# aszepieniec/stark-brainfuck

Hardware: AMD Instinct MI355X
Metric: goldilocks_ntt_field_elements_per_sec (higher is better)
Workload: dtype u64 (mod 2^64-2^32+1); 1 GPU; forward NTT of 8 independent 2^24-point base-field columns resident in HBM (BASELINE config 5); log_n=24, total_columns=8

## Files before the change

### stark_brainfuck_amd/csrc/ntt.hip

```cpp
#include <cstdio>
#include <cstdlib>
#include <cstring>
#include <vector>

#define BFS_GL_SUB4
#include "runtime.hpp"

namespace bfs {

template <int B1, int B2, int B3, int LOGC, int MODE, bool NT>
__global__ void __launch_bounds__(256) ntt_tile_kernel(const PassArgs a) {
    extern __shared__ __attribute__((aligned(16))) u64 smem[];
    typedef TileCfg<B1, B2, B3, LOGC, MODE> Cfg;
    u64* tw = smem + (B2 > 0 ? ((Cfg::LDS_WORDS + 1) & ~1) : 0);
    static_assert(B1 == 4, "one sub-group of 16 elements per thread");
    constexpr u32 TW_N = Cfg::U >= 2 ? (1u << (B1 + B2)) : 0;
    const u64* tab = a.tw1;
    const u32 tw_shift = a.tb.t_in_log - (B1 + B2);
    const u32 tid = threadIdx.x;
    const u64* lrow = tile_load_row<Cfg, LOGC, MODE>(a, blockIdx.x);
    const u64* srow_g = tile_store_row<Cfg, LOGC, MODE>(a, blockIdx.x);
    const u64* row = lrow ? lrow : srow_g;
    const bool has_row = row != nullptr;
    u64 tw0 = 0, rw0 = 0;
    if (TW_N && tid < TW_N) tw0 = tab[(u64)tid << tw_shift];
    if (has_row && tid < (1u << Cfg::S)) rw0 = row[tid];
    u64 x[16];
    ntt_stage1_load<B1, B2, B3, LOGC, MODE, NT>(a, tid, blockIdx.x, blockIdx.y, 0, x);
    u64* rw = tw + Cfg::TW_WORDS;
    if (TW_N && tid < TW_N) tw[tid] = tw0;
    if (has_row && tid < (1u << Cfg::S)) rw[tid] = rw0;
    for (u32 i = tid + blockDim.x; i < TW_N; i += blockDim.x) tw[i] = tab[(u64)i << tw_shift];
    if (has_row)
        for (u32 i = tid + blockDim.x; i < (1u << Cfg::S); i += blockDim.x) rw[i] = row[i];
    const u64* rowtw = lrow ? rw : nullptr;
    const u64* srow = srow_g && !lrow ? rw : nullptr;
    if (Cfg::U >= 2 || has_row) __syncthreads();
    ntt_stage1_compute<B1, B2, B3, LOGC, MODE, NT>(a, smem, tw, rowtw, threadIdx.x, blockIdx.x, blockIdx.y, 0, x, srow);
    if constexpr (B2 > 0) {
        __syncthreads();
        ntt_stage2<B1, B2, B3, LOGC, MODE, NT>(a, smem, threadIdx.x, blockIdx.x, blockIdx.y, srow);
    }
    if constexpr (B3 > 0) {
        __syncthreads();
        ntt_stage3<B1, B2, B3, LOGC, MODE, NT>(a, smem, threadIdx.x, blockIdx.x, blockIdx.y, srow);
    }
}

#ifndef BFS_NTT_SPLIT_WAVES
#define BFS_NTT_SPLIT_WAVES 6
#endif
template <int B1, int B2, int B3, int LOGC, int MODE, bool NT>
__global__ void __launch_bounds__(256, B2 >= 3 ? BFS_NTT_SPLIT_WAVES : 0) ntt_tile_kernel_split(const PassArgs a) {
    static_assert(B1 == 4 && B2 > 0 && B3 == 0, "two register stages, 16 elements per thread");
    extern __shared__ __attribute__((aligned(16))) u64 smem[];
    typedef TileCfg<B1, B2, B3, LOGC, MODE> Cfg;
    constexpr u32 TILE_BYTES = (Cfg::LDS_WORDS * 4 + 15) & ~15u;
    u32* tile = (u32*)smem;
    u64* tw = (u64*)((char*)smem + TILE_BYTES);
    constexpr u32 TW_N = 1u << (B1 + B2);
    const u64* tab = a.tw1;
    const u32 tw_shift = a.tb.t_in_log - (B1 + B2);
    const u32 tid = threadIdx.x;
    const u32 bx = blockIdx.x, by = blockIdx.y;
    const u64* lrow = tile_load_row<Cfg, LOGC, MODE>(a, bx);
    const u64* srow_g = tile_store_row<Cfg, LOGC, MODE>(a, bx);
    const u64* row = lrow ? lrow : srow_g;
    const bool has_row = row != nullptr;
    u64 tw0 = 0, rw0 = 0;
    if (tid < TW_N) tw0 = tab[(u64)tid << tw_shift];
    if (has_row && tid < (1u << Cfg::S)) rw0 = row[tid];
    u64 x[16];
    ntt_stage1_load<B1, B2, B3, LOGC, MODE, NT>(a, tid, bx, by, 0, x);
    u64* rw = tw + Cfg::TW_WORDS;
    if (tid < TW_N) tw[tid] = tw0;
// ... 12 lines not shown
        for (int d = 0; d < Q2; ++d) lo[s * Q2 + d] = tile[stage2_in_index<B1, B2, B3, LOGC, MODE>(tid, s, d)];
    __syncthreads();
    BFS_UNROLL
    for (int m = 0; m < 16; ++m) tile[stage1_out_index<B1, B2, B3, LOGC, MODE>(a, tid, 0, m)] = (u32)(x[m] >> 32);
    __syncthreads();
    BFS_UNROLL
    for (int s = 0; s < SG2; ++s) {
        u64 y[Q2];
        BFS_UNROLL
        for (int d = 0; d < Q2; ++d) y[d] = ((u64)tile[stage2_in_index<B1, B2, B3, LOGC, MODE>(tid, s, d)] << 32) | lo[s * Q2 + d];
        ntt_stage2_from<B1, B2, B3, LOGC, MODE, NT>(a, smem, tid, bx, by, s, y, srow);
    }
}

__global__ void ntt_small_kernel(const SmallArgs a) { ntt_small_body(a, threadIdx.x, blockIdx.y); }

template <int B1, int B2, int B3, int LOGC, int MODE>
static int launch_tile(TileShape<B1, B2, B3, LOGC, MODE>, const PassArgs& a, u32 grid_x, u32 batch, hipStream_t stream) {
    typedef TileCfg<B1, B2, B3, LOGC, MODE> Cfg;
    const size_t row_words = (a.tb.row != nullptr || a.tb.srow != nullptr) ? (1u << Cfg::S) : 0;
    if constexpr (MODE == PASS_SINGLE) {
        const size_t lds = (size_t)((B2 > 0 ? ((Cfg::LDS_WORDS + 1) & ~1) + Cfg::TW_WORDS : 0) + row_words) * sizeof(u64);
        if (a.streaming)
            hipLaunchKernelGGL((ntt_tile_kernel<B1, B2, B3, LOGC, MODE, true>), dim3(grid_x, batch), dim3(Cfg::W), lds, stream, a);
        else
            hipLaunchKernelGGL((ntt_tile_kernel<B1, B2, B3, LOGC, MODE, false>), dim3(grid_x, batch), dim3(Cfg::W), lds, stream, a);
    } else {
        const size_t lds = ((Cfg::LDS_WORDS * 4 + 15) & ~15u) + (Cfg::TW_WORDS + row_words) * sizeof(u64);
        if (a.streaming)
            hipLaunchKernelGGL((ntt_tile_kernel_split<B1, B2, B3, LOGC, MODE, true>), dim3(grid_x, batch), dim3(Cfg::W), lds, stream, a);
        else
            hipLaunchKernelGGL((ntt_tile_kernel_split<B1, B2, B3, LOGC, MODE, false>), dim3(grid_x, batch), dim3(Cfg::W), lds, stream, a);
    }
    BFS_HIP(hipGetLastError());
    return BFS_OK;
}

enum { TBL_W_LO = 1, TBL_W_HI, TBL_T_IN, TBL_T_IN_LAST, TBL_S_LO, TBL_S_HI, TBL_ROW };

static int get_row_tables(const NttPlan& p, u32 t, u64 root, const u64** d_row, const u64** d_srow) {
    *d_row = nullptr;
    *d_srow = nullptr;
    NttRowSpec load, store;
    ntt_row_specs(p, t, root, load, store);
    for (int which = 0; which < 2; ++which) {
        const NttRowSpec& sp = which ? store : load;
        if (sp.omega == 0) continue;
        const u64** out = which ? d_srow : d_row;
        const u64 key = ((u64)sp.a_bits << 24) | ((u64)sp.b_bits << 16) | TBL_ROW;
        if (cached_table_lookup(sp.omega, key, 0, out)) continue;
        std::vector<u64> host;
        ntt_product_table(sp.omega, sp.a_bits, sp.b_bits, host);
        BFS_TRY(cached_table(sp.omega, key, 0, host.data(), host.size(), out));
    }
    return BFS_OK;
// ... 15 lines not shown
        BFS_TRY(cached_table(root, kb | TBL_T_IN, 0, ht.t_in.data(), ht.t_in.size(), &tb.t_in));
        BFS_TRY(cached_table(root, kb | TBL_T_IN_LAST, post_scale, ht.t_in_last.data(), ht.t_in_last.size(), &tb.t_in_last));
    }
    if (shift != 1) {
        if (!(cached_table_lookup(shift, kb | TBL_S_LO, 0, &tb.s_lo) && cached_table_lookup(shift, kb | TBL_S_HI, 0, &tb.s_hi))) {
            CosetHostTables ct;
            ntt_build_coset_tables(p, shift, ct);
            BFS_TRY(cached_table(shift, kb | TBL_S_LO, 0, ct.s_lo.data(), ct.s_lo.size(), &tb.s_lo));
            BFS_TRY(cached_table(shift, kb | TBL_S_HI, 0, ct.s_hi.data(), ct.s_hi.size(), &tb.s_hi));
        }
    }
    return BFS_OK;
}

int ntt_power_tables(u64 root, u32 log_n, const u64** lo, const u64** hi, u32* lo_bits) {
    NttPlan p;
    if (!ntt_make_plan(log_n, root, p)) { set_error("no table plan for log_n = %u", log_n); return BFS_ERR_BAD_ARG; }
    NttTables tb;
    BFS_TRY(get_tables(p, root, 1, 1, tb));
    *lo = tb.w_lo; *hi = tb.w_hi; *lo_bits = tb.lo_bits;
    return BFS_OK;
}

int ntt_run_steps(const NttCall& c, const NttPlan& p, u64* mid, u32 first, u32 last) {
    NttTables tb;
    BFS_TRY(get_tables(p, c.root, c.shift, c.post_scale, tb));
    const NttSchedule s = ntt_make_schedule(p, c.n_in, mid != nullptr);
    const struct { u64* ptr; u64 stride; } buf[3] = {{const_cast<u64*>(c.in), c.in_stride}, {c.out, c.out_stride}, {mid, 1ull << p.log_n}};
    for (u32 k = first; k <= last && k < s.nsteps; ++k) {
        const NttStep& st = s.step[k];
        BFS_TRY(get_row_tables(p, st.pass, c.root, &tb.row, &tb.srow));
        PassArgs a = ntt_pass_args(p, st.pass, buf[st.src].ptr, buf[st.dst].ptr, buf[st.src].stride, buf[st.dst].stride, st.count, tb, c.shift != 1, c.shift, c.post_scale);
        a.streaming = c.streaming;
        const int rc = ntt_with_tile_shape(st.mode, st.S, [&](auto shape) { return launch_tile(shape, a, st.grid_x, c.batch, c.stream); });
        if (rc == BFS_ERR_BAD_ARG) set_error("internal: no tile kernel for a %u-bit digit in mode %u", st.S, st.mode);
        BFS_TRY(rc);
    }
    return BFS_OK;
}

const NttEnv& ntt_env() {
    static const NttEnv env = [] {
        NttEnv v{NttRouteMode::Remembered, NTT_ROUTE_DIRECT, false, -1, true, false};
        if (const char* e = getenv("BFS_NTT_WS_PROBE")) {
            if (e[0] == '0' || !strcmp(e, "direct")) v.route_mode = NttRouteMode::Forced;
            else if (!strncmp(e, "buffer", 6) && e[6] >= '0' && e[6] < '0' + NTT_ROUTE_CANDIDATES && !e[7]) { v.route_mode = NttRouteMode::Forced; v.forced_route = e[6] - '0'; }
            else if (!strcmp(e, "auto") || !strcmp(e, "1")) v.route_mode = NttRouteMode::Auto;
        }
        if (const char* e = getenv("BFS_NTT_WS_PROBE_LOG")) v.probe_log = e[0] == '1';
        if (const char* e = getenv("BFS_NTT_STREAMING")) v.force_streaming = atoi(e);
        if (const char* e = getenv("BFS_NTT_EXPAND")) v.allow_expand = e[0] != '0';
        v.plan_log = getenv("BFS_NTT_PLAN_LOG") != nullptr;
        return v;
    }();
    return env;
}

int ntt_launch(const u64* d_in, u64 n_in, u64 in_stride, u64* d_out, u64 out_stride, u32 log_n, u32 batch, u64 root,
               u64 shift, u64 post_scale, hipStream_t stream) {
    if (log_n > 32) { set_error("field has no 2^%u-th root of unity (algebra.py:124-125)", log_n); return BFS_ERR_BAD_ARG; }
    const u64 n = 1ull << log_n;
    if (n_in > n) { set_error("more coefficients (%llu) than the evaluation order (%llu)", (unsigned long long)n_in, (unsigned long long)n); return BFS_ERR_TOO_MANY_COEFFS; }
    if (batch == 0) return BFS_OK;
    if (d_out == nullptr || (d_in == nullptr && n_in != 0)) { set_error("bfs_gl_ntt: null device pointer"); return BFS_ERR_BAD_ARG; }
    if (batch > 1 && (out_stride < n || in_stride < n_in)) {
        set_error("bfs_gl_ntt: transforms of a batch overlap (in_stride %llu < %llu coefficients or out_stride %llu < n = %llu)",
                  (unsigned long long)in_stride, (unsigned long long)n_in, (unsigned long long)out_stride, (unsigned long long)n);
        return BFS_ERR_BAD_ARG;
    }
    if (log_n <= NTT_TILE_LOG && n_in != 0) {
        if (ntt_buffers_overlap(d_in, n_in, in_stride, d_out, n, out_stride, batch) && !(d_in == d_out && in_stride == out_stride)) {
            void* w = nullptr;
            const size_t span = (size_t)((u64)(batch - 1) * in_stride + n_in) * sizeof(u64);
            BFS_TRY(workspace(0, span, stream, &w));
            BFS_HIP(hipMemcpyAsync(w, d_in, span, hipMemcpyDeviceToDevice, stream));
// ... 2 lines not shown
    }
    if (batch > 65535) {
        for (u32 done = 0; done < batch;) {
            const u32 part = batch - done < 65535 ? batch - done : 65535;
            BFS_TRY(ntt_launch(d_in + (u64)done * in_stride, n_in, in_stride, d_out + (u64)done * out_stride, out_stride, log_n, part, root,
                               shift, post_scale, stream));
            done += part;
        }
        return BFS_OK;
    }
    int rc = ntt_check_root(root, log_n);
    if (rc == BFS_ERR_NOT_ROOT) { set_error("primitive root must be nth root of unity, where n is %llu", (unsigned long long)n); return rc; }
    if (rc == BFS_ERR_NOT_PRIMITIVE) { set_error("primitive root %llu is not primitive nth root of unity, where n is %llu", (unsigned long long)root, (unsigned long long)n); return rc; }
    const NttEnv& env = ntt_env();
    const bool overlap = log_n > NTT_TILE_LOG && n_in != 0 && ntt_buffers_overlap(d_in, n_in, in_stride, d_out, n, out_stride, batch);
    NttPlan p;
    if (!ntt_choose_plan(log_n, n_in, root, overlap, env.allow_expand, p)) { set_error("no NTT plan for log_n = %u", log_n); return BFS_ERR_BAD_ARG; }
    if (p.npass == 0) {
        SmallArgs a{d_in, d_out, in_stride, out_stride, n_in, log_n, root, shift, post_scale};
        hipLaunchKernelGGL(ntt_small_kernel, dim3(1, batch), dim3(64), 0, stream, a);
        BFS_HIP(hipGetLastError());
        return BFS_OK;
    }
    const u32 streaming = env.force_streaming >= 0 ? (u32)(env.force_streaming != 0) : (u32)((u64)n * batch * sizeof(u64) > NTT_STREAMING_BYTES);
    const NttCall c{d_in, n_in, in_stride, d_out, out_stride, batch, root, shift, post_scale, streaming, stream};
    if (env.plan_log) fprintf(stderr, "ntt plan: log_n %u n_in %llu batch %u overlap %d allow %d in %p out %p\n", log_n, (unsigned long long)n_in, batch, (int)overlap, (int)env.allow_expand, (const void*)d_in, (void*)d_out);
    int route = NTT_ROUTE_DIRECT;
    if (!overlap && !p.expand && p.npass > 1) BFS_TRY(ntt_route(c, p, &route));
    u64* mid = nullptr;
    if (overlap || route >= 0) {
        void* w = nullptr;
        BFS_TRY(workspace(route >= 0 ? NTT_ROUTE_SLOT0 + route : 0, (size_t)n * batch * sizeof(u64), stream, &w));
        mid = (u64*)w;
    }
    return ntt_run_steps(c, p, mid, 0, 3);
}

}
```

### stark_brainfuck_amd/csrc/ntt_core.hpp

```cpp
#pragma once
#include "gl.hpp"

namespace bfs {

constexpr u64 cx_mulmod(u64 a, u64 b) { return (u64)(((u128)a * b) % GL_P); }
constexpr u64 cx_pow2(int k) {
    u64 r = 1;
    for (int i = 0; i < k; ++i) r = cx_mulmod(r, 2);
    return r;
}

template <int K>
BFS_HD u64 mul_pow2(u64 x) {
    static_assert(K >= 0 && K < 96, "rotation amount");
    constexpr int q = K / 32, r = K % 32;
    if constexpr (K == 0) {
        return x;
    } else if constexpr (q == 0) {
        return gl_reduce96((u32)(x >> (64 - r)), x << r);
    } else {
        const u32 x0 = (u32)x, x1 = (u32)(x >> 32);
        u32 y0 = x0, y1 = x1, y2 = 0;
        if constexpr (r != 0) {
            y0 = x0 << r;
// ... 42 lines not shown
}
template <int Q, int LIVE, bool OUT_LAZY>
BFS_HD void dif_sparse(u64* x) {
    if constexpr (Q >= 2) {
        if constexpr (LIVE > Q / 2) {
            dif<Q, OUT_LAZY>(x);
        } else {
            dif_sparse_level<Q, LIVE, OUT_LAZY>(x);
            dif_sparse<Q / 2, LIVE, OUT_LAZY>(x);
            dif_sparse<Q / 2, LIVE, OUT_LAZY>(x + Q / 2);
        }
    }
}

constexpr u32 cx_bitrev(u32 v, int bits) {
    u32 r = 0;
    for (int i = 0; i < bits; ++i) r |= ((v >> i) & 1u) << (bits - 1 - i);
    return r;
}

template <int BITS>
BFS_HD u32 perm_digit(int m, u32 uinv) { return (cx_bitrev((u32)m, BITS) * uinv) & ((1u << BITS) - 1); }

template <bool NT>
BFS_HD u64 ntt_ld(const u64* p) {
#if defined(__HIP_DEVICE_COMPILE__)
    if constexpr (NT) return __builtin_nontemporal_load(p);
#endif
    return *p;
}
template <bool NT>
BFS_HD void ntt_st(u64* p, u64 v) {
#if defined(__HIP_DEVICE_COMPILE__)
    if constexpr (NT) { __builtin_nontemporal_store(v, p); return; }
#endif
    *p = v;
}

struct NttTables {
    const u64* w_lo;
    const u64* w_hi;
    u32 lo_bits;
    u32 t_in_log;
    const u64* t_in;
    const u64* t_in_last;
    const u64* s_lo;
    const u64* s_hi;
    const u64* row;
    const u64* srow;
};

enum { PASS_COLUMN = 0, PASS_SINGLE = 1, PASS_FIRST = 2, PASS_EXPAND = 3 };

struct PassArgs {
    const u64* in;
    u64* out;
    u64 in_batch_stride, out_batch_stride;
// ... 111 lines not shown
template <typename Cfg, int LOGC, int MODE>
BFS_HD const u64* tile_store_row(const PassArgs& a, u32 bid_x) {
    if constexpr (MODE != PASS_FIRST) return nullptr;
    if (a.tb.srow == nullptr) return nullptr;
    const u64 c0 = (u64)(bid_x & ((1u << a.lognl) - 1)) << LOGC;
    const u64 j1 = c0 >> (a.logL - pass_bits_of(a.pass_bits, 1));
    return a.tb.srow + (j1 << Cfg::S);
}

template <int B1, int B2, int B3, int LOGC, int MODE>
BFS_HD void stage2_pos(u32 G, u32& c, u32& f1, u32& f3) {
    if constexpr (MODE == PASS_FIRST) {
        f1 = G & ((1u << B1) - 1);
        c = (G >> B1) & ((1u << LOGC) - 1);
        f3 = G >> (B1 + LOGC);
    } else {
        c = G & ((1u << LOGC) - 1);
        const u32 rest = G >> LOGC;
        f1 = rest & ((1u << B1) - 1);
        f3 = rest >> B1;
    }
}

template <typename Cfg, int LOGC, int MODE, int BQ, bool NT = false>
BFS_HD void final_store(const PassArgs& a, const TileGeom& g, const u64* x, u32 klow, int kshift, u32 c, const u64* srow = nullptr) {
    constexpr int Q = 1 << BQ;
    const bool scale = (Cfg::U == 1) && a.post_scale != 1;
    u64* tp;
    u32 step_log;
    if constexpr (MODE == PASS_COLUMN || MODE == PASS_EXPAND) {
        tp = g.out + g.row0 + ((u64)klow << a.logL) + c;
        step_log = (u32)kshift + a.logL;
    } else if constexpr (MODE == PASS_FIRST) {
        tp = g.out + (digit_reverse(g.c0 + c, a.pass_bits, 1, (int)a.npass - 1) << Cfg::S) + klow;
        step_log = (u32)kshift;
    } else {
        tp = g.out + klow;
        step_log = (u32)kshift;
    }
    BFS_UNROLL
    for (int m = 0; m < Q; ++m) {
        u64 v = scale ? gl_mul(x[m], a.post_scale) : x[m];
        if (srow != nullptr) v = gl_mul(v, srow[klow + (perm_digit<BQ>(m, a.uinv) << kshift)]);
        ntt_st<NT>(tp + ((u64)perm_digit<BQ>(m, a.uinv) << step_log), v);
    }
}

// ... 7 lines not shown
template <int B1, int B2, int B3, int LOGC, int MODE>
BFS_HD void stage1_oc(u32 tid, int sub, u32& o, u32& c) {
    typedef TileCfg<B1, B2, B3, LOGC, MODE> Cfg;
    const u32 G = (u32)sub * Cfg::W + tid;
    c = G & ((1u << LOGC) - 1);
    o = G >> LOGC;
}

template <int B1, int B2, int B3, int LOGC, int MODE>
BFS_HD Stage1Pos<B1, B2, B3, LOGC, MODE> stage1_pos(const PassArgs& a, const TileGeom& g, u32 tid, int sub) {
    typedef TileCfg<B1, B2, B3, LOGC, MODE> Cfg;
    Stage1Pos<B1, B2, B3, LOGC, MODE> p;
    stage1_oc<B1, B2, B3, LOGC, MODE>(tid, sub, p.o, p.c);
    if constexpr (MODE != PASS_SINGLE) {
        p.idx0 = g.row0 + ((u64)p.o << a.logL) + p.c;
        p.step_log = Cfg::SH1 + a.logL;
    } else {
        p.idx0 = p.o;
        p.step_log = Cfg::SH1;
    }
    return p;
}

template <int B1, int B2, int B3, int LOGC, int MODE, bool NT = false>
BFS_HD void ntt_stage1_load(const PassArgs& a, u32 tid, u32 bid_x, u32 bid_y, int sub, u64* x) {
    typedef TileCfg<B1, B2, B3, LOGC, MODE> Cfg;
    constexpr int Q = 1 << B1;
    const TileGeom g = tile_geom<Cfg, LOGC, MODE>(a, bid_x, bid_y);
    const Stage1Pos<B1, B2, B3, LOGC, MODE> p = stage1_pos<B1, B2, B3, LOGC, MODE>(a, g, tid, sub);
    if constexpr (MODE == PASS_EXPAND) {
        const u64 i0 = ((u64)p.o << a.tw_shift) + g.h;
        const u32 sl = Cfg::SH1 + a.tw_shift;
        const u64* ip = a.in + (u64)bid_y * a.in_batch_stride + i0;
        BFS_UNROLL
        for (int d = 0; d < Q; ++d) x[d] = (i0 + ((u64)d << sl) < a.n_main) ? ntt_ld<NT>(ip + ((u64)d << sl)) : 0;
        return;
    }
    const u64* tp = g.in + p.idx0;
    if (a.partial) {
        BFS_UNROLL
        for (int d = 0; d < Q; ++d) x[d] = (p.idx0 + ((u64)d << p.step_log) < a.n_in) ? ntt_ld<NT>(tp + ((u64)d << p.step_log)) : 0;
    } else {
        BFS_UNROLL
        for (int d = 0; d < Q; ++d) x[d] = ntt_ld<NT>(tp + ((u64)d << p.step_log));
    }
}

template <int B1, int B2, int B3, int LOGC, int MODE>
BFS_HD u32 stage1_out_index(const PassArgs& a, u32 tid, int sub, int m) {
    typedef TileCfg<B1, B2, B3, LOGC, MODE> Cfg;
    u32 o, c;
    stage1_oc<B1, B2, B3, LOGC, MODE>(tid, sub, o, c);
    return lds_addr<Cfg, LOGC>((perm_digit<B1>(m, a.uinv) << Cfg::SH1) | o, c);
}

template <int B1, int B2, int B3, int LOGC, int MODE>
BFS_HD u32 stage2_in_index(u32 tid, int s, int d) {
    typedef TileCfg<B1, B2, B3, LOGC, MODE> Cfg;
    u32 c, f1, f3;
    stage2_pos<B1, B2, B3, LOGC, MODE>((u32)s * Cfg::W + tid, c, f1, f3);
    return lds_addr<Cfg, LOGC>((f1 << Cfg::SH1) | ((u32)d << Cfg::SH2) | f3, c);
}

template <int B1, int B2, int B3, int LOGC, int MODE, bool NT = false>
BFS_HD void ntt_stage1_values(const PassArgs& a, const u64* tw, const u64* rowtw, u32 tid, u32 bid_x, u32 bid_y, int sub, u64* x,
                              const u64* srow = nullptr) {
    typedef TileCfg<B1, B2, B3, LOGC, MODE> Cfg;
    constexpr int Q = 1 << B1;
    const TileGeom g = tile_geom<Cfg, LOGC, MODE>(a, bid_x, bid_y);
    const u64 nmask = (1ull << a.log_n) - 1;
    const Stage1Pos<B1, B2, B3, LOGC, MODE> p = stage1_pos<B1, B2, B3, LOGC, MODE>(a, g, tid, sub);
    const u32 o = p.o, c = p.c;
    u32 dmax = Q;
    if constexpr (MODE == PASS_EXPAND) {
        const u32 sl = Cfg::SH1 + a.tw_shift;
        const u64 live = (a.n_main + ((1ull << sl) - 1)) >> sl;
        if (live < (u64)Q) dmax = (u32)live;
    } else if (a.partial) {
        const u64 live = (a.n_in + ((1ull << p.step_log) - 1)) >> p.step_log;
        if (live < (u64)Q) dmax = (u32)live;
    }
    if constexpr (MODE == PASS_EXPAND) {
        const u64 i0 = ((u64)o << a.tw_shift) + g.h;
        if (a.extras != 0 && i0 < (u64)a.extras) {
            const u64 e = g.in[(1ull << a.main_bits) + i0];
            u64 f = tw_pow(a.tb.w_lo, a.tb.w_hi, a.tb.lo_bits, ((g.c0 + c) << a.main_bits) & nmask);
            if (a.has_coset) f = gl_mul(f, a.extra_scale);
// ... 37 lines not shown
            if (dmax <= 1) dif_sparse<16, 1, (Cfg::U >= 2)>(x);
            else if (dmax <= 2) dif_sparse<16, 2, (Cfg::U >= 2)>(x);
            else if (dmax <= 4) dif_sparse<16, 4, (Cfg::U >= 2)>(x);
            else dif_sparse<16, 8, (Cfg::U >= 2)>(x);
        }
    } else {
        dif<Q, (Cfg::U >= 2)>(x);
    }
    if constexpr (Cfg::U == 1) {
        final_store<Cfg, LOGC, MODE, B1, NT>(a, g, x, 0, 0, c, srow);
    } else {
        const u32 i2 = o >> B3;
        BFS_UNROLL
        for (int m = 0; m < Q; ++m) {
            const u32 k1 = perm_digit<B1>(m, a.uinv);
            const u32 e = mul24(i2, k1) & ((1u << (B1 + B2)) - 1);
            const bool unit = (m == 0) && a.unit0;
            if (!unit) x[m] = gl_mul(x[m], tw[e]);
            else x[m] = gl_canon(x[m]);
        }
    }
}

template <int B1, int B2, int B3, int LOGC, int MODE, bool NT = false>
BFS_HD void ntt_stage1_compute(const PassArgs& a, u64* smem, const u64* tw, const u64* rowtw, u32 tid, u32 bid_x, u32 bid_y, int sub, u64* x,
                               const u64* srow = nullptr) {
    typedef TileCfg<B1, B2, B3, LOGC, MODE> Cfg;
    ntt_stage1_values<B1, B2, B3, LOGC, MODE, NT>(a, tw, rowtw, tid, bid_x, bid_y, sub, x, srow);
    if constexpr (Cfg::U >= 2) {
        BFS_UNROLL
        for (int m = 0; m < (1 << B1); ++m) smem[stage1_out_index<B1, B2, B3, LOGC, MODE>(a, tid, sub, m)] = x[m];
    }
}

template <int B1, int B2, int B3, int LOGC, int MODE>
BFS_HD void ntt_stage1(const PassArgs& a, u64* smem, const u64* tw, const u64* rowtw, u32 tid, u32 bid_x, u32 bid_y, const u64* srow = nullptr) {
    constexpr int Q = 1 << B1, SG = 16 / Q;
    BFS_UNROLL
    for (int s = 0; s < SG; ++s) {
        u64 x[Q];
        ntt_stage1_load<B1, B2, B3, LOGC, MODE>(a, tid, bid_x, bid_y, s, x);
        ntt_stage1_compute<B1, B2, B3, LOGC, MODE>(a, smem, tw, rowtw, tid, bid_x, bid_y, s, x, srow);
    }
}

template <int B1, int B2, int B3, int LOGC, int MODE, bool NT = false>
BFS_HD void ntt_stage2_from(const PassArgs& a, u64* smem, u32 tid, u32 bid_x, u32 bid_y, int s, u64* x, const u64* srow = nullptr) {
    typedef TileCfg<B1, B2, B3, LOGC, MODE> Cfg;
    if constexpr (B2 > 0) {
        constexpr int Q = 1 << B2;
        const TileGeom g = tile_geom<Cfg, LOGC, MODE>(a, bid_x, bid_y);
        u32 c, f1, f3;
        stage2_pos<B1, B2, B3, LOGC, MODE>((u32)s * Cfg::W + tid, c, f1, f3);
        dif<Q, (Cfg::U == 3 || MODE == PASS_FIRST)>(x);
        if constexpr (Cfg::U == 2) {
            final_store<Cfg, LOGC, MODE, B2, NT>(a, g, x, f1, B1, c, srow);
        } else {
            BFS_UNROLL
            for (int m = 0; m < Q; ++m) {
                const u32 k2 = perm_digit<B2>(m, a.uinv);
                const u32 e = mul24(f3, f1 + (k2 << B1)) & ((1u << Cfg::S) - 1);
                const u64 v = gl_mul(x[m], a.tw2[(u64)e << (a.tb.t_in_log - Cfg::S)]);
                smem[lds_addr<Cfg, LOGC>((f1 << Cfg::SH1) | (k2 << Cfg::SH2) | f3, c)] = v;
            }
        }
    }
}

template <int B1, int B2, int B3, int LOGC, int MODE, bool NT = false>
BFS_HD void ntt_stage2(const PassArgs& a, u64* smem, u32 tid, u32 bid_x, u32 bid_y, const u64* srow = nullptr) {
    if constexpr (B2 > 0) {
        constexpr int Q = 1 << B2, SG = 16 / Q;
        BFS_UNROLL
        for (int s = 0; s < SG; ++s) {
            u64 x[Q];
            BFS_UNROLL
            for (int d = 0; d < Q; ++d) x[d] = smem[stage2_in_index<B1, B2, B3, LOGC, MODE>(tid, s, d)];
            ntt_stage2_from<B1, B2, B3, LOGC, MODE, NT>(a, smem, tid, bid_x, bid_y, s, x, srow);
        }
    }
}

template <int B1, int B2, int B3, int LOGC, int MODE, bool NT = false>
BFS_HD void ntt_stage3(const PassArgs& a, u64* smem, u32 tid, u32 bid_x, u32 bid_y, const u64* srow = nullptr) {
    typedef TileCfg<B1, B2, B3, LOGC, MODE> Cfg;
    if constexpr (B3 > 0) {
        constexpr int Q = 1 << B3, SG = 16 / Q;
        const TileGeom g = tile_geom<Cfg, LOGC, MODE>(a, bid_x, bid_y);
        BFS_UNROLL
        for (int s = 0; s < SG; ++s) {
            const u32 G = (u32)s * Cfg::W + tid;
            const u32 c = G & ((1u << LOGC) - 1);
            const u32 rest = G >> LOGC;
            const u32 f1 = rest & ((1u << B1) - 1), f2 = rest >> B1;
            u64 x[Q];
            BFS_UNROLL
            for (int d = 0; d < Q; ++d) x[d] = smem[lds_addr<Cfg, LOGC>((f1 << Cfg::SH1) | (f2 << Cfg::SH2) | (u32)d, c)];
            dif<Q>(x);
            final_store<Cfg, LOGC, MODE, B3, NT>(a, g, x, f1 + (f2 << B1), B1 + B2, c, srow);
        }
    }
}

struct SmallArgs {
    const u64* in;
    u64* out;
// ... 23 lines not shown
```

### stark_brainfuck_amd/csrc/ntt_route.cpp

```cpp
#include <algorithm>
#include <cstdio>
#include <map>
#include <mutex>
#include <set>
#include <string>
#include <tuple>
#include <vector>

#include "runtime.hpp"

namespace bfs {

constexpr int NTT_ROUTE_SIGHTINGS = 3;
#ifndef NTT_ROUTE_WARM
#define NTT_ROUTE_WARM 10
#define NTT_ROUTE_REPS 8
#endif
constexpr u64 NTT_ROUTE_MIN_BYTES = 256ull << 20;
constexpr int ROUTE_UNSEEN = -100;
namespace {
std::mutex g_route_mu;
struct RouteKey {
    int dev; hipStream_t stream; const void* in; const void* out; u64 in_stride, out_stride, shape; u64 in_bytes, out_bytes;
    bool operator<(const RouteKey& o) const {
// ... 183 lines not shown
        if (ROUTE_UNSEEN - --state < NTT_ROUTE_SIGHTINGS) return BFS_OK;
    }
    return ntt_measure_route(c, p, key, route);
}

int ntt_tune(const u64* d_in, u64 in_stride, u64* d_out, u64 out_stride, u32 log_n, u32 batch, u64 root, hipStream_t stream, int* route_out) {
    if (route_out) *route_out = NTT_ROUTE_DIRECT;
    if (log_n > 32 || batch == 0 || batch > 65535 || d_in == nullptr || d_out == nullptr) { set_error("bfs_ntt_tune: bad argument"); return BFS_ERR_BAD_ARG; }
    const u64 n = 1ull << log_n;
    if (batch > 1 && (out_stride < n || in_stride < n)) { set_error("bfs_ntt_tune: transforms of a batch overlap"); return BFS_ERR_BAD_ARG; }
    int rc = ntt_check_root(root, log_n);
    if (rc != BFS_OK) { set_error("bfs_ntt_tune: the root is not a primitive 2^%u-th root of unity", log_n); return rc; }
    NttPlan p;
    if (!ntt_make_plan(log_n, root, p)) { set_error("no NTT plan for log_n = %u", log_n); return BFS_ERR_BAD_ARG; }
    if (p.npass < 2 || ntt_buffers_overlap(d_in, n, in_stride, d_out, n, out_stride, batch) || ntt_env().route_mode == NttRouteMode::Forced ||
        (u64)n * batch * sizeof(u64) < NTT_ROUTE_MIN_BYTES)
        return BFS_OK;
    hipStreamCaptureStatus cap = hipStreamCaptureStatusNone;
    if (hipStreamIsCapturing(stream, &cap) == hipSuccess && cap != hipStreamCaptureStatusNone) {
        set_error("bfs_ntt_tune: the stream is being captured (the measurement synchronises it)");
        return BFS_ERR_BAD_ARG;
    }
    (void)hipGetLastError();
    const NttCall c{d_in, n, in_stride, d_out, out_stride, batch, root, 1, 1, (u32)((u64)n * batch * sizeof(u64) > NTT_STREAMING_BYTES), stream};
    int dev = 0;
    BFS_HIP(hipGetDevice(&dev));
    int route = NTT_ROUTE_DIRECT;
    BFS_TRY(ntt_measure_route(c, p, route_key(dev, c, log_n), &route));
    if (route_out) *route_out = route;
    return BFS_OK;
}

}
```

### stark_brainfuck_amd/csrc/runtime.cpp

```cpp
#include "runtime.hpp"

#include <cstdarg>
#include <cstdio>
#include <cstdlib>
#include <cstring>
#include <map>
#include <mutex>
#include <tuple>
#include <unordered_map>
#include <vector>

namespace bfs {

static thread_local char g_error[512] = "";

void set_error(const char* fmt, ...) {
    va_list ap;
    va_start(ap, fmt);
    vsnprintf(g_error, sizeof g_error, fmt, ap);
    va_end(ap);
}

const char* last_error() { return g_error; }

namespace {
struct Scratch {
    void* ptr = nullptr;
    size_t bytes = 0;
};
std::mutex g_mu;
std::map<std::tuple<int, hipStream_t, int>, Scratch> g_scratch;
std::map<std::tuple<int, uint64_t, uint64_t, uint64_t>, const u64*> g_tables;
constexpr size_t TABLE_CAP = 4096;
std::vector<std::pair<int, const u64*>> g_retired_tables;

void retire_tables_locked() {
    (void)hipDeviceSynchronize();
    int cur = 0;
    (void)hipGetDevice(&cur);
    for (auto& t : g_retired_tables) {
        if (hipSetDevice(t.first) == hipSuccess) { (void)hipDeviceSynchronize(); (void)hipFree((void*)t.second); }
    }
    (void)hipSetDevice(cur);
    g_retired_tables.clear();
    for (auto& kv : g_tables) g_retired_tables.emplace_back(std::get<0>(kv.first), kv.second);
    g_tables.clear();
}
}

namespace {
size_t size_class(size_t bytes) {
    if (bytes <= 256) return 256;
    size_t p = 256;
    while (p < bytes) p <<= 1;
// ... 206 lines not shown
            BFS_HIP(hipStreamSynchronize(stream));
            BFS_HIP(hipFree(s.ptr));
            s.ptr = nullptr;
            s.bytes = 0;
        }
        BFS_HIP(hipMalloc(&s.ptr, bytes));
        s.bytes = bytes;
    }
    *out = s.ptr;
    return BFS_OK;
}

bool workspace_peek(int slot, hipStream_t stream, void** ptr, size_t* bytes) {
    int dev = 0;
    if (hipGetDevice(&dev) != hipSuccess) return false;
    std::lock_guard<std::mutex> lock(g_mu);
    auto it = g_scratch.find(std::make_tuple(dev, stream, slot));
    if (it == g_scratch.end() || !it->second.ptr) return false;
    if (ptr) *ptr = it->second.ptr;
    if (bytes) *bytes = it->second.bytes;
    return true;
}

int workspace_release(int slot, hipStream_t stream) {
    int dev = 0;
    BFS_HIP(hipGetDevice(&dev));
    std::lock_guard<std::mutex> lock(g_mu);
    auto it = g_scratch.find(std::make_tuple(dev, stream, slot));
    if (it != g_scratch.end()) {
        if (it->second.ptr) (void)hipFree(it->second.ptr);
        g_scratch.erase(it);
    }
    return BFS_OK;
}

int stream_retire(hipStream_t stream) {
    BFS_HIP(hipStreamSynchronize(stream));
    int dev = 0;
    BFS_HIP(hipGetDevice(&dev));
    {
        std::lock_guard<std::mutex> lock(g_mu);
        for (auto it = g_scratch.begin(); it != g_scratch.end();) {
            if (std::get<0>(it->first) == dev && std::get<1>(it->first) == stream) {
                if (it->second.ptr) (void)hipFree(it->second.ptr);
                it = g_scratch.erase(it);
            } else {
                ++it;
            }
        }
    }
    for (Pool* pool : {&g_device_pool, &g_host_pool}) {
        std::lock_guard<std::mutex> lock(pool->mu);
        for (auto& kv : pool->free_lists)
            for (Block& b : kv.second)
                if (b.released_on == stream) b.released_on = NO_STREAM;
    }
    return BFS_OK;
}

bool cached_table_lookup(uint64_t a, uint64_t b, uint64_t c, const u64** d_out) {
    int dev = 0;
    if (hipGetDevice(&dev) != hipSuccess) return false;
    std::lock_guard<std::mutex> lock(g_mu);
    auto it = g_tables.find(std::make_tuple(dev, a, b, c));
// ... 30 lines not shown
```

### stark_brainfuck_amd/csrc/runtime.hpp

```cpp
#pragma once
#include <hip/hip_runtime.h>
#include <stddef.h>
#include <stdint.h>

#include <type_traits>

#include "ntt_plan.hpp"

namespace bfs {

void set_error(const char* fmt, ...) __attribute__((format(printf, 1, 2)));
const char* last_error();

#define BFS_HIP(expr)                                                                                   \
    do {                                                                                                \
        hipError_t e_ = (expr);                                                                         \
        if (e_ != hipSuccess) {                                                                         \
            ::bfs::set_error("%s failed: %s (%s:%d)", #expr, hipGetErrorString(e_), __FILE__, __LINE__); \
            return BFS_ERR_HIP;                                                                         \
        }                                                                                               \
    } while (0)

#define BFS_TRY(expr)            \
    do {                         \
        int rc_ = (expr);        \
        if (rc_) return rc_;     \
    } while (0)

int workspace(int slot, size_t bytes, hipStream_t stream, void** out);
int workspace_release(int slot, hipStream_t stream);
bool workspace_peek(int slot, hipStream_t stream, void** ptr, size_t* bytes);

static const hipStream_t NO_STREAM = (hipStream_t)(uintptr_t)-1;
int device_alloc(size_t bytes, hipStream_t stream, void** out);
int device_release(void* ptr, hipStream_t stream);
int device_pool_trim();
void device_pool_stats(size_t* live_bytes, size_t* cached_bytes);
int host_alloc(size_t bytes, void** out);
int host_release(void* ptr);

int copy_h2d(void* d, const void* h, size_t bytes, hipStream_t stream);
int copy_d2h(void* h, const void* d, size_t bytes, hipStream_t stream);

int stream_retire(hipStream_t stream);

int cached_table(uint64_t key_a, uint64_t key_b, uint64_t key_c, const u64* host, size_t count, const u64** d_out);
bool cached_table_lookup(uint64_t key_a, uint64_t key_b, uint64_t key_c, const u64** d_out);

struct FriFoldArgs {
    const u64* in;
    u64 in_stride, half;
    Xfe alpha[3];
    u64 scal[7];
    const u64* winv_lo;
    const u64* winv_hi;
    u32 lo_bits, round_shift;
    u32 log2_folding;
};
inline void fri_fold_constants(FriFoldArgs& f, u32 k, u64 n, const Xfe& alpha, u64 offset, u64 omega) {
    f.log2_folding = k;
    f.half = n >> k;
    f.alpha[0] = alpha;
    for (u32 j = 1; j < 3; ++j) f.alpha[j] = j < k ? xfe_mul(f.alpha[j - 1], f.alpha[j - 1]) : Xfe{{0, 0, 0}};
    u64 gj = gl_mul(gl_inv(2), gl_inv(offset));
    u64 zj = k > 1 ? gl_pow(gl_inv(omega), f.half) : 1;
// ... 54 lines not shown
}
constexpr u64 FRI_FUSED_MAX = 16384;
int merkle_build_xfe_fold_launch(const FriFoldArgs& fold, u64* d_cw, u64 cw_stride, u64 n, u64* d_nodes, hipStream_t stream, u64* root_out, u64 seq);
int fri_round_fused_launch(const FriFoldArgs& fold, u64* d_cw, u64 cw_stride, u64 n, u64* d_nodes, hipStream_t stream, u64* root_out, u64 seq);

struct NttCall {
    const u64* in;
    u64 n_in, in_stride;
    u64* out;
    u64 out_stride;
    u32 batch;
    u64 root, shift, post_scale;
    u32 streaming;
    hipStream_t stream;
};
constexpr u64 NTT_STREAMING_BYTES = 128ull << 20;
int ntt_launch(const u64* d_in, u64 n_in, u64 in_stride, u64* d_out, u64 out_stride, u32 log_n, u32 batch, u64 root,
               u64 shift, u64 post_scale, hipStream_t stream);
int ntt_run_steps(const NttCall& c, const NttPlan& p, u64* mid, u32 first, u32 last);
int ntt_power_tables(u64 root, u32 log_n, const u64** lo, const u64** hi, u32* lo_bits);
constexpr int NTT_ROUTE_CANDIDATES = 3;
constexpr int NTT_ROUTE_DIRECT = -1;
enum class NttRouteMode { Remembered, Auto, Forced };
struct NttEnv {
    NttRouteMode route_mode;
    int forced_route;
    bool probe_log;
    int force_streaming;
    bool allow_expand;
    bool plan_log;
};
const NttEnv& ntt_env();

constexpr int NTT_ROUTE_SLOT0 = 16;
int ntt_route(const NttCall& c, const NttPlan& p, int* route);
int ntt_route_probe_info(float* us, int* route, unsigned long long* probes);
int ntt_tune(const u64* d_in, u64 in_stride, u64* d_out, u64 out_stride, u32 log_n, u32 batch, u64 root, hipStream_t stream, int* route_out);
size_t ntt_route_forget_range(const void* lo, size_t bytes, bool may_free);
void ntt_route_trim();

int mul_pointwise_launch(const u64* a, const u64* b, u64* out, u64 n, hipStream_t stream);
int batch_inverse_launch(const u64* in, u64* out, u64 n, hipStream_t stream);
int scale_launch(const u64* in, u64* out, u64 n, u64 stride, u32 batch, u64 factor, hipStream_t stream);
int xfe_mul_pointwise_launch(const u64* a, u64 a_stride, const u64* b, u64 b_stride, u64* out, u64 out_stride, u64 n, hipStream_t stream);
int xfe_batch_inverse_launch(const u64* in, u64 in_stride, u64* out, u64 out_stride, u64 n, hipStream_t stream);

int merkle_inner_launch(u64* d_nodes, u32 depth, u64 n_leaves, hipStream_t stream, u64* root_out = nullptr, u64 seq = 0);
int merkle_build_xfe_launch(const u64* d_limbs, u64 limb_stride, u64 n, u64* d_nodes, hipStream_t stream, u64* root_out = nullptr, u64 seq = 0);
int merkle_build_bfe_launch(const u64* d_values, u64 n, u64* d_nodes, hipStream_t stream);
int merkle_build_bytes_launch(const u64* d_data, const u64* d_offsets, const u32* d_lengths, u64 n, u64* d_nodes, hipStream_t stream);

int coset_tree_launch(const FriFoldArgs* fold, u64* d_cw, u64 cw_stride, u64 q, u32 log2_coset, u64* d_nodes, hipStream_t stream, u64* not_mine,
                      u64 token, u64* root_out, u64 seq);
// ... 21 lines not shown
```

Baseline: 103.0 billion elements/s.

## Pipeline batched NTT columns across two streams with per-pass nontemporal hints

For batched NTTs of mid-size columns (64–128 MiB each, three passes), the batch is now split into single-column runs that alternate between the caller's stream and a helper stream, joined with events. The goal is to overlap the passes of neighbouring columns and keep each column's working set closer to cache. Nontemporal hints are split into separate load and store flags: first-pass loads from the input use nontemporal loads while the other passes use regular accesses, and row tables are fetched once per call instead of once per step. In exchange there are more kernel launches, a lazily created helper stream, and possible contention between the two streams.

```diff
diff --git a/stark_brainfuck_amd/csrc/ntt.hip b/stark_brainfuck_amd/csrc/ntt.hip
--- a/stark_brainfuck_amd/csrc/ntt.hip
+++ b/stark_brainfuck_amd/csrc/ntt.hip
@@ -8,7 +8,7 @@
 
 namespace bfs {
 
-template <int B1, int B2, int B3, int LOGC, int MODE, bool NT>
+template <int B1, int B2, int B3, int LOGC, int MODE, int NT>
 __global__ void __launch_bounds__(256) ntt_tile_kernel(const PassArgs a) {
     extern __shared__ __attribute__((aligned(16))) u64 smem[];
     typedef TileCfg<B1, B2, B3, LOGC, MODE> Cfg;
@@ -50,7 +50,7 @@
 #ifndef BFS_NTT_SPLIT_WAVES
 #define BFS_NTT_SPLIT_WAVES 6
 #endif
-template <int B1, int B2, int B3, int LOGC, int MODE, bool NT>
+template <int B1, int B2, int B3, int LOGC, int MODE, int NT>
 __global__ void __launch_bounds__(256, B2 >= 3 ? BFS_NTT_SPLIT_WAVES : 0) ntt_tile_kernel_split(const PassArgs a) {
     static_assert(B1 == 4 && B2 > 0 && B3 == 0, "two register stages, 16 elements per thread");
     extern __shared__ __attribute__((aligned(16))) u64 smem[];
@@ -109,15 +109,18 @@
     if constexpr (MODE == PASS_SINGLE) {
         const size_t lds = (size_t)((B2 > 0 ? ((Cfg::LDS_WORDS + 1) & ~1) + Cfg::TW_WORDS : 0) + row_words) * sizeof(u64);
         if (a.streaming)
-            hipLaunchKernelGGL((ntt_tile_kernel<B1, B2, B3, LOGC, MODE, true>), dim3(grid_x, batch), dim3(Cfg::W), lds, stream, a);
+            hipLaunchKernelGGL((ntt_tile_kernel<B1, B2, B3, LOGC, MODE, NTT_NT_ALL>), dim3(grid_x, batch), dim3(Cfg::W), lds, stream, a);
         else
-            hipLaunchKernelGGL((ntt_tile_kernel<B1, B2, B3, LOGC, MODE, false>), dim3(grid_x, batch), dim3(Cfg::W), lds, stream, a);
+            hipLaunchKernelGGL((ntt_tile_kernel<B1, B2, B3, LOGC, MODE, NTT_NT_NONE>), dim3(grid_x, batch), dim3(Cfg::W), lds, stream, a);
     } else {
         const size_t lds = ((Cfg::LDS_WORDS * 4 + 15) & ~15u) + (Cfg::TW_WORDS + row_words) * sizeof(u64);
-        if (a.streaming)
-            hipLaunchKernelGGL((ntt_tile_kernel_split<B1, B2, B3, LOGC, MODE, true>), dim3(grid_x, batch), dim3(Cfg::W), lds, stream, a);
+        constexpr int NT_FIRST = MODE == PASS_FIRST ? NTT_NT_LOADS : NTT_NT_ALL;
+        if (a.streaming == NT_FIRST)
+            hipLaunchKernelGGL((ntt_tile_kernel_split<B1, B2, B3, LOGC, MODE, NT_FIRST>), dim3(grid_x, batch), dim3(Cfg::W), lds, stream, a);
+        else if (a.streaming)
+            hipLaunchKernelGGL((ntt_tile_kernel_split<B1, B2, B3, LOGC, MODE, NTT_NT_ALL>), dim3(grid_x, batch), dim3(Cfg::W), lds, stream, a);
         else
-            hipLaunchKernelGGL((ntt_tile_kernel_split<B1, B2, B3, LOGC, MODE, false>), dim3(grid_x, batch), dim3(Cfg::W), lds, stream, a);
+            hipLaunchKernelGGL((ntt_tile_kernel_split<B1, B2, B3, LOGC, MODE, NTT_NT_NONE>), dim3(grid_x, batch), dim3(Cfg::W), lds, stream, a);
     }
     BFS_HIP(hipGetLastError());
     return BFS_OK;
@@ -179,26 +182,67 @@
     return BFS_OK;
 }
 
-int ntt_run_steps(const NttCall& c, const NttPlan& p, u64* mid, u32 first, u32 last) {
+struct NttCallTables {
     NttTables tb;
-    BFS_TRY(get_tables(p, c.root, c.shift, c.post_scale, tb));
+    const u64* row[4];
+    const u64* srow[4];
+};
+static int get_call_tables(const NttCall& c, const NttPlan& p, NttCallTables& t) {
+    BFS_TRY(get_tables(p, c.root, c.shift, c.post_scale, t.tb));
+    for (u32 pass = p.expand ? 1 : 0; pass < p.npass && pass < 4; ++pass) BFS_TRY(get_row_tables(p, pass, c.root, &t.row[pass], &t.srow[pass]));
+    return BFS_OK;
+}
+static int run_steps(const NttCall& c, const NttPlan& p, u64* mid, u32 first, u32 last, const NttCallTables& t, u32 nt_in) {
     const NttSchedule s = ntt_make_schedule(p, c.n_in, mid != nullptr);
     const struct { u64* ptr; u64 stride; } buf[3] = {{const_cast<u64*>(c.in), c.in_stride}, {c.out, c.out_stride}, {mid, 1ull << p.log_n}};
+    NttTables tb = t.tb;
     for (u32 k = first; k <= last && k < s.nsteps; ++k) {
         const NttStep& st = s.step[k];
-        BFS_TRY(get_row_tables(p, st.pass, c.root, &tb.row, &tb.srow));
+        tb.row = t.row[st.pass];
+        tb.srow = t.srow[st.pass];
         PassArgs a = ntt_pass_args(p, st.pass, buf[st.src].ptr, buf[st.dst].ptr, buf[st.src].stride, buf[st.dst].stride, st.count, tb, c.shift != 1, c.shift, c.post_scale);
-        a.streaming = c.streaming;
+        a.streaming = st.src == NTT_BUF_IN ? nt_in : c.streaming;
         const int rc = ntt_with_tile_shape(st.mode, st.S, [&](auto shape) { return launch_tile(shape, a, st.grid_x, c.batch, c.stream); });
         if (rc == BFS_ERR_BAD_ARG) set_error("internal: no tile kernel for a %u-bit digit in mode %u", st.S, st.mode);
         BFS_TRY(rc);
     }
     return BFS_OK;
 }
+int ntt_run_steps(const NttCall& c, const NttPlan& p, u64* mid, u32 first, u32 last) {
+    NttCallTables t;
+    BFS_TRY(get_call_tables(c, p, t));
+    return run_steps(c, p, mid, first, last, t, c.streaming);
+}
+
+static int ntt_run_columns(const NttCall& c, const NttPlan& p) {
+    const NttEnv& env = ntt_env();
+    StreamPair sp;
+    BFS_TRY(stream_pair(c.stream, &sp));
+    NttCallTables t;
+    BFS_TRY(get_call_tables(c, p, t));
+    const u32 nt_rest = env.force_streaming > 0 ? NTT_NT_ALL : NTT_NT_NONE;
+    const u32 nt_in = env.force_streaming >= 0 ? nt_rest : NTT_NT_LOADS;
+    BFS_HIP(hipEventRecord(sp.fork, c.stream));
+    BFS_HIP(hipStreamWaitEvent(sp.helper, sp.fork, 0));
+    int rc = BFS_OK;
+    for (u32 col = 0; rc == BFS_OK && col < c.batch; ++col) {
+        NttCall one = c;
+        one.in = c.in + (u64)col * c.in_stride;
+        one.out = c.out + (u64)col * c.out_stride;
+        one.batch = 1;
+        one.streaming = nt_rest;
+        one.stream = (col & 1) ? sp.helper : c.stream;
+        rc = run_steps(one, p, nullptr, 0, 3, t, nt_in);
+    }
+    if (hipEventRecord(sp.join, sp.helper) != hipSuccess || hipStreamWaitEvent(c.stream, sp.join, 0) != hipSuccess) {
+        if (rc == BFS_OK) { set_error("bfs_gl_ntt: joining the column pipeline's second stream failed"); rc = BFS_ERR_HIP; }
+    }
+    return rc;
+}
 
 const NttEnv& ntt_env() {
     static const NttEnv env = [] {
-        NttEnv v{NttRouteMode::Remembered, NTT_ROUTE_DIRECT, false, -1, true, false};
+        NttEnv v{NttRouteMode::Remembered, NTT_ROUTE_DIRECT, false, -1, true, false, NttPipeline::BySize};
         if (const char* e = getenv("BFS_NTT_WS_PROBE")) {
             if (e[0] == '0' || !strcmp(e, "direct")) v.route_mode = NttRouteMode::Forced;
             else if (!strncmp(e, "buffer", 6) && e[6] >= '0' && e[6] < '0' + NTT_ROUTE_CANDIDATES && !e[7]) { v.route_mode = NttRouteMode::Forced; v.forced_route = e[6] - '0'; }
@@ -208,6 +252,7 @@
         if (const char* e = getenv("BFS_NTT_STREAMING")) v.force_streaming = atoi(e);
         if (const char* e = getenv("BFS_NTT_EXPAND")) v.allow_expand = e[0] != '0';
         v.plan_log = getenv("BFS_NTT_PLAN_LOG") != nullptr;
+        if (const char* e = getenv("BFS_NTT_PIPELINE")) v.pipeline = !strcmp(e, "force") ? NttPipeline::Forced : e[0] == '0' ? NttPipeline::Off : NttPipeline::BySize;
         return v;
     }();
     return env;
@@ -256,11 +301,21 @@
         BFS_HIP(hipGetLastError());
         return BFS_OK;
     }
-    const u32 streaming = env.force_streaming >= 0 ? (u32)(env.force_streaming != 0) : (u32)((u64)n * batch * sizeof(u64) > NTT_STREAMING_BYTES);
+    const bool nt = env.force_streaming >= 0 ? env.force_streaming != 0 : (u64)n * batch * sizeof(u64) > NTT_STREAMING_BYTES;
+    const u32 streaming = nt ? NTT_NT_ALL : NTT_NT_NONE;
     const NttCall c{d_in, n_in, in_stride, d_out, out_stride, batch, root, shift, post_scale, streaming, stream};
     if (env.plan_log) fprintf(stderr, "ntt plan: log_n %u n_in %llu batch %u overlap %d allow %d in %p out %p\n", log_n, (unsigned long long)n_in, batch, (int)overlap, (int)env.allow_expand, (const void*)d_in, (void*)d_out);
     int route = NTT_ROUTE_DIRECT;
     if (!overlap && !p.expand && p.npass > 1) BFS_TRY(ntt_route(c, p, &route));
+    bool columns = batch >= 2 && !overlap && !p.expand && n_in == n && env.pipeline != NttPipeline::Off &&
+                   (env.pipeline == NttPipeline::Forced ? p.npass >= 2 : p.npass == 3 && n * sizeof(u64) >= NTT_PIPELINE_MIN_BYTES && n * sizeof(u64) <= NTT_PIPELINE_MAX_BYTES);
+    if (columns) {
+        hipStreamCaptureStatus cap = hipStreamCaptureStatusNone;
+        if (hipStreamIsCapturing(stream, &cap) != hipSuccess) { (void)hipGetLastError(); columns = false; }
+        else if (cap != hipStreamCaptureStatusNone) columns = false;
+    }
+    if (env.plan_log) fprintf(stderr, "ntt route: %s\n", columns ? "pipelined columns" : overlap ? "staged" : p.expand ? "expansion" : route >= 0 ? "single launch via buffer" : "single launch");
+    if (columns) return ntt_run_columns(c, p);
     u64* mid = nullptr;
     if (overlap || route >= 0) {
         void* w = nullptr;
diff --git a/stark_brainfuck_amd/csrc/ntt_core.hpp b/stark_brainfuck_amd/csrc/ntt_core.hpp
--- a/stark_brainfuck_amd/csrc/ntt_core.hpp
+++ b/stark_brainfuck_amd/csrc/ntt_core.hpp
@@ -88,17 +88,18 @@
 template <int BITS>
 BFS_HD u32 perm_digit(int m, u32 uinv) { return (cx_bitrev((u32)m, BITS) * uinv) & ((1u << BITS) - 1); }
 
-template <bool NT>
+enum { NTT_NT_NONE = 0, NTT_NT_LOADS = 1, NTT_NT_STORES = 2, NTT_NT_ALL = 3 };
+template <int NT>
 BFS_HD u64 ntt_ld(const u64* p) {
 #if defined(__HIP_DEVICE_COMPILE__)
-    if constexpr (NT) return __builtin_nontemporal_load(p);
+    if constexpr ((NT & NTT_NT_LOADS) != 0) return __builtin_nontemporal_load(p);
 #endif
     return *p;
 }
-template <bool NT>
+template <int NT>
 BFS_HD void ntt_st(u64* p, u64 v) {
 #if defined(__HIP_DEVICE_COMPILE__)
-    if constexpr (NT) { __builtin_nontemporal_store(v, p); return; }
+    if constexpr ((NT & NTT_NT_STORES) != 0) { __builtin_nontemporal_store(v, p); return; }
 #endif
     *p = v;
 }
@@ -256,7 +257,7 @@
     }
 }
 
-template <typename Cfg, int LOGC, int MODE, int BQ, bool NT = false>
+template <typename Cfg, int LOGC, int MODE, int BQ, int NT = 0>
 BFS_HD void final_store(const PassArgs& a, const TileGeom& g, const u64* x, u32 klow, int kshift, u32 c, const u64* srow = nullptr) {
     constexpr int Q = 1 << BQ;
     const bool scale = (Cfg::U == 1) && a.post_scale != 1;
@@ -310,7 +311,7 @@
     return p;
 }
 
-template <int B1, int B2, int B3, int LOGC, int MODE, bool NT = false>
+template <int B1, int B2, int B3, int LOGC, int MODE, int NT = 0>
 BFS_HD void ntt_stage1_load(const PassArgs& a, u32 tid, u32 bid_x, u32 bid_y, int sub, u64* x) {
     typedef TileCfg<B1, B2, B3, LOGC, MODE> Cfg;
     constexpr int Q = 1 << B1;
@@ -350,7 +351,7 @@
     return lds_addr<Cfg, LOGC>((f1 << Cfg::SH1) | ((u32)d << Cfg::SH2) | f3, c);
 }
 
-template <int B1, int B2, int B3, int LOGC, int MODE, bool NT = false>
+template <int B1, int B2, int B3, int LOGC, int MODE, int NT = 0>
 BFS_HD void ntt_stage1_values(const PassArgs& a, const u64* tw, const u64* rowtw, u32 tid, u32 bid_x, u32 bid_y, int sub, u64* x,
                               const u64* srow = nullptr) {
     typedef TileCfg<B1, B2, B3, LOGC, MODE> Cfg;
@@ -434,7 +435,7 @@
     }
 }
 
-template <int B1, int B2, int B3, int LOGC, int MODE, bool NT = false>
+template <int B1, int B2, int B3, int LOGC, int MODE, int NT = 0>
 BFS_HD void ntt_stage1_compute(const PassArgs& a, u64* smem, const u64* tw, const u64* rowtw, u32 tid, u32 bid_x, u32 bid_y, int sub, u64* x,
                                const u64* srow = nullptr) {
     typedef TileCfg<B1, B2, B3, LOGC, MODE> Cfg;
@@ -456,7 +457,7 @@
     }
 }
 
-template <int B1, int B2, int B3, int LOGC, int MODE, bool NT = false>
+template <int B1, int B2, int B3, int LOGC, int MODE, int NT = 0>
 BFS_HD void ntt_stage2_from(const PassArgs& a, u64* smem, u32 tid, u32 bid_x, u32 bid_y, int s, u64* x, const u64* srow = nullptr) {
     typedef TileCfg<B1, B2, B3, LOGC, MODE> Cfg;
     if constexpr (B2 > 0) {
@@ -479,7 +480,7 @@
     }
 }
 
-template <int B1, int B2, int B3, int LOGC, int MODE, bool NT = false>
+template <int B1, int B2, int B3, int LOGC, int MODE, int NT = 0>
 BFS_HD void ntt_stage2(const PassArgs& a, u64* smem, u32 tid, u32 bid_x, u32 bid_y, const u64* srow = nullptr) {
     if constexpr (B2 > 0) {
         constexpr int Q = 1 << B2, SG = 16 / Q;
@@ -493,7 +494,7 @@
     }
 }
 
-template <int B1, int B2, int B3, int LOGC, int MODE, bool NT = false>
+template <int B1, int B2, int B3, int LOGC, int MODE, int NT = 0>
 BFS_HD void ntt_stage3(const PassArgs& a, u64* smem, u32 tid, u32 bid_x, u32 bid_y, const u64* srow = nullptr) {
     typedef TileCfg<B1, B2, B3, LOGC, MODE> Cfg;
     if constexpr (B3 > 0) {
diff --git a/stark_brainfuck_amd/csrc/ntt_route.cpp b/stark_brainfuck_amd/csrc/ntt_route.cpp
--- a/stark_brainfuck_amd/csrc/ntt_route.cpp
+++ b/stark_brainfuck_amd/csrc/ntt_route.cpp
@@ -229,7 +229,7 @@
         return BFS_ERR_BAD_ARG;
     }
     (void)hipGetLastError();
-    const NttCall c{d_in, n, in_stride, d_out, out_stride, batch, root, 1, 1, (u32)((u64)n * batch * sizeof(u64) > NTT_STREAMING_BYTES), stream};
+    const NttCall c{d_in, n, in_stride, d_out, out_stride, batch, root, 1, 1, (u64)n * batch * sizeof(u64) > NTT_STREAMING_BYTES ? (u32)NTT_NT_ALL : (u32)NTT_NT_NONE, stream};
     int dev = 0;
     BFS_HIP(hipGetDevice(&dev));
     int route = NTT_ROUTE_DIRECT;
diff --git a/stark_brainfuck_amd/csrc/runtime.cpp b/stark_brainfuck_amd/csrc/runtime.cpp
--- a/stark_brainfuck_amd/csrc/runtime.cpp
+++ b/stark_brainfuck_amd/csrc/runtime.cpp
@@ -30,6 +30,12 @@
 };
 std::mutex g_mu;
 std::map<std::tuple<int, hipStream_t, int>, Scratch> g_scratch;
+std::map<std::pair<int, hipStream_t>, StreamPair> g_stream_pairs;
+void destroy_stream_pair(const StreamPair& sp) {
+    if (sp.fork) (void)hipEventDestroy(sp.fork);
+    if (sp.join) (void)hipEventDestroy(sp.join);
+    if (sp.helper) (void)hipStreamDestroy(sp.helper);
+}
 std::map<std::tuple<int, uint64_t, uint64_t, uint64_t>, const u64*> g_tables;
 constexpr size_t TABLE_CAP = 4096;
 std::vector<std::pair<int, const u64*>> g_retired_tables;
@@ -282,6 +288,27 @@
     return true;
 }
 
+int stream_pair(hipStream_t stream, StreamPair* out) {
+    int dev = 0;
+    BFS_HIP(hipGetDevice(&dev));
+    std::lock_guard<std::mutex> lock(g_mu);
+    auto it = g_stream_pairs.find(std::make_pair(dev, stream));
+    if (it == g_stream_pairs.end()) {
+        StreamPair sp{nullptr, nullptr, nullptr};
+        hipError_t e = hipStreamCreateWithFlags(&sp.helper, hipStreamNonBlocking);
+        if (e == hipSuccess) e = hipEventCreateWithFlags(&sp.fork, hipEventDisableTiming);
+        if (e == hipSuccess) e = hipEventCreateWithFlags(&sp.join, hipEventDisableTiming);
+        if (e != hipSuccess) {
+            destroy_stream_pair(sp);
+            set_error("creating the library's second stream failed: %s", hipGetErrorString(e));
+            return BFS_ERR_HIP;
+        }
+        it = g_stream_pairs.emplace(std::make_pair(dev, stream), sp).first;
+    }
+    *out = it->second;
+    return BFS_OK;
+}
+
 int workspace_release(int slot, hipStream_t stream) {
     int dev = 0;
     BFS_HIP(hipGetDevice(&dev));
@@ -300,6 +327,11 @@
     BFS_HIP(hipGetDevice(&dev));
     {
         std::lock_guard<std::mutex> lock(g_mu);
+        auto sp = g_stream_pairs.find(std::make_pair(dev, stream));
+        if (sp != g_stream_pairs.end()) {
+            destroy_stream_pair(sp->second);
+            g_stream_pairs.erase(sp);
+        }
         for (auto it = g_scratch.begin(); it != g_scratch.end();) {
             if (std::get<0>(it->first) == dev && std::get<1>(it->first) == stream) {
                 if (it->second.ptr) (void)hipFree(it->second.ptr);
diff --git a/stark_brainfuck_amd/csrc/runtime.hpp b/stark_brainfuck_amd/csrc/runtime.hpp
--- a/stark_brainfuck_amd/csrc/runtime.hpp
+++ b/stark_brainfuck_amd/csrc/runtime.hpp
@@ -41,6 +41,12 @@
 
 int copy_h2d(void* d, const void* h, size_t bytes, hipStream_t stream);
 int copy_d2h(void* h, const void* d, size_t bytes, hipStream_t stream);
+
+struct StreamPair {
+    hipStream_t helper;
+    hipEvent_t fork, join;
+};
+int stream_pair(hipStream_t stream, StreamPair* out);
 
 int stream_retire(hipStream_t stream);
 
@@ -141,6 +147,9 @@
 constexpr int NTT_ROUTE_CANDIDATES = 3;
 constexpr int NTT_ROUTE_DIRECT = -1;
 enum class NttRouteMode { Remembered, Auto, Forced };
+enum class NttPipeline { Off, BySize, Forced };
+constexpr u64 NTT_PIPELINE_MIN_BYTES = 64ull << 20;
+constexpr u64 NTT_PIPELINE_MAX_BYTES = 128ull << 20;
 struct NttEnv {
     NttRouteMode route_mode;
     int forced_route;
@@ -148,6 +157,7 @@
     int force_streaming;
     bool allow_expand;
     bool plan_log;
+    NttPipeline pipeline;
 };
 const NttEnv& ntt_env();
 
```

Measured after the change: 106.6 billion elements/s (median of 6 runs). +3.5%, better.
